# ssghost/SymbolicRegression.jl

Measured on AMD Instinct MI355X. Metric: node·row evals/sec (Float32, 4096 trees×1M rows) at 1/2/4/8 GPUs; % VALU peak, higher is better.
Workload: dtype f32

## Files before the change

symbolicregression.jl_amd/csrc/jit.cpp:

```cpp
#include "jit.h"

#include <elf.h>

#include <algorithm>
#include <chrono>
#include <cmath>
#include <cstdarg>
#include <cstdio>
#include <cstdlib>
#include <cstring>
#include <atomic>
#include <functional>
#include <mutex>
#include <thread>
#include <unordered_map>

#include "jit_asm.h"

#define HIP_CHECK(expr)                                                                  \
  do {                                                                                   \
    hipError_t _e = (expr);                                                              \
    if (_e != hipSuccess)                                                                \
      throw Error(SRHIP_ERR_DEVICE, std::string(#expr) + ": " + hipGetErrorString(_e));  \
  } while (0)
// ... 240 lines not shown
}

struct Gen {
  Asm& as;
  const Tmpl& T;
  uint64_t base_va;
  bool fast_opt;
  std::vector<IrOp> ops;
  Opnd root;
  bool fast = false;
  bool g_can = false, g_min = false, g_exp = false, g_trig = false, has_trig = false, has_call = false;
  enum { L_NONE = -1, L_A = 100, L_B = 101 };
  std::vector<int> loc;
  int pool_owner[NPOOL];
  int a_owner = -1, b_owner = -1;
  int xblk[256];
  int xlast[256];
  bool xinl[256];
  bool xdirect = false;
  std::vector<int> feats;
  int load_idx[256];
  int nloads = 0, waited = 0;
  std::vector<int> next_call;
  int L_tile = -1, L_done = -1, L_redo = -1, L_bail = -1;
  std::string why;
  bool out = false;
  int out_rreg = -1;
  int gbase = 1 << 30;
  bool gwaited = true;
  int gidx[256];
  int gnum = 0, gdone = 0;
  bool gany = false;
  bool gprefetch = [] { const char* e = std::getenv("SRHIP_JIT_GPREFETCH"); return e && e[0] == '1'; }();
  int L_reload = -1;
  void emit_gloads() {
    as.vop2(VOP2_LSHLREV_B32, "v_lshlrev_b32_e32", VGT, K(2), VLANE4);
    as.sop2(SOP2_LSHL_B32, "s_lshl_b32", 0, S(S_TILE), K(10));
    as.sop2(SOP2_ADD_U32, "s_add_u32", 0, S(S_GCOL), S(0));
    as.sop2(SOP2_ADDC_U32, "s_addc_u32", 1, S(S_GCOL + 1), K(0));
    for (size_t j = 0; j < feats.size(); ++j) {
      const int f = feats[j];
      if (!is_g(f)) continue;
      const uint32_t g = (uint32_t)(f - gbase);
      int sb = 0;
      if (g > 0) {
        as.sop2(SOP2_MUL_I32, "s_mul_i32", 2, S(S_GSTRIDE), K(g));
        as.sop2(SOP2_MUL_HI_U32, "s_mul_hi_u32", 3, S(S_GSTRIDE), K(g));
// ... 6 lines not shown
  }
  static constexpr int S_GCOL = 36, S_GSTRIDE = 38;
  bool is_g(int v) const { return v >= gbase; }

  bool trig_full = false;
  bool manual_off = false;
  bool off_exp = false, off_trig = false, off_div = false;
  static int div_rk() {
    static const int r = [] {
      for (int k = 0; k < kNumRoutines; ++k)
        if (std::string(kRoutineName[k]) == "b_div_rk") return k;
      return -1;
    }();
    return r;
  }
  static int full_routine(int rid) {
    const std::string want = std::string(kRoutineName[rid]) + "_full";
    for (int k = 0; k < kNumRoutines; ++k)
      if (want == kRoutineName[k]) return k;
    return rid;
  }
  bool inline_ok = false;
  bool packed = true, pkmov = true;
  static constexpr int SC0 = 24, NSC = 16, SPROG = 56;
  bool memc = false;
  int loss = SRHIP_LOSS_L2;
  uint64_t lparam = 0;
  std::vector<int> cpcs;
  int cslot(const Opnd& q) {
    for (size_t k = 0; k < cpcs.size(); ++k)
      if (cpcs[k] == q.pc) return (int)k;
    cpcs.push_back(q.pc);
    return (int)cpcs.size() - 1;
  }
  int creg(const Opnd& q) const {
    for (size_t k = 0; k < cpcs.size(); ++k)
      if (cpcs[k] == q.pc) return SC0 + (int)k;
    throw Error(SRHIP_ERR_INVALID, "jit: constant without a slot");
  }
  Gen(Asm& a, const Tmpl& t, uint64_t va, bool f) : as(a), T(t), base_va(va), fast_opt(f) {
    const char* e = std::getenv("SRHIP_JIT_INLINE");
    inline_ok = e && e[0] == '1';
    const char* xd = std::getenv("SRHIP_JIT_XDIRECT");
    xdirect = !(xd && xd[0] == '0');
    const char* pk = std::getenv("SRHIP_JIT_PACKED");
    packed = !(pk && pk[0] == '0');
    const char* pm = std::getenv("SRHIP_JIT_PKMOV");
    pkmov = !(pm && pm[0] == '0');
    const char* tf = std::getenv("SRHIP_JIT_TRIG_FULL");
    trig_full = tf && tf[0] == '1';
    const char* mo = std::getenv("SRHIP_JIT_MANUAL");
    manual_off = mo && mo[0] == '0';
    if (const char* mf = std::getenv("SRHIP_JIT_MANUAL_OFF")) {
      const std::string l(mf);
      off_exp = l.find("exp") != std::string::npos;
      off_trig = l.find("trig") != std::string::npos;
      off_div = l.find("div") != std::string::npos;
    }
  }

  uint64_t cur_va() const { return base_va + as.bytes(); }
  static bool trig_guard_on() {
    static const bool on = [] { const char* e = std::getenv("SRHIP_JIT_TRIG_GUARD"); return !(e && e[0] == '0'); }();
    return on;
  }
  bool trig_of_tainted(const IrOp& o) const {
    static const bool zs_only = [] { const char* e = std::getenv("SRHIP_JIT_TRIG_GUARD_ZS"); return e && e[0] == '1'; }();
    return o.un && (o.op == SRHIP_UOP_SIN || o.op == SRHIP_UOP_COS) && o.a.k == O_VAL && ops[o.a.v].taint &&
           (o.zs || !zs_only);
  }
  static bool loss_guards_on() {
    static const bool on = [] { const char* e = std::getenv("SRHIP_JIT_LOSS_GUARDS"); return !(e && e[0] == '0'); }();
    return on;
  }
  static uint32_t can_eps_bits() {
// ... 566 lines not shown
      ++nloads;
    }
    for (size_t j = 0; j < feats.size(); ++j) {
      const int f = feats[j];
      pool_owner[j] = 1000 + f;
      if (is_g(f)) continue;
      load_idx[f] = nloads++;
      as.ds_read_b128(VPOOL0 + R * (int)j, VLANE, (1 + f) * TILE * 4);
    }
    gwaited = !gany;
    gdone = 0;
    std::fill(loc.begin(), loc.end(), (int)L_NONE);
    for (int i = 0; i < (int)ops.size(); ++i) {
      if (ops[i].rid >= 0) { if (!emit_call(i)) return false; }
      else if (!emit_inline(i)) return false;
    }
    int rreg;
    if (root.k == O_VAL) rreg = reg_of_loc(loc[root.v]);
    else if (root.k == O_X) { wait_for(root); rreg = VPOOL0 + R * xblk[root.v]; }
    else {
      for (int e = 0; e < R; ++e) as.vop1(VOP1_MOV, "v_mov_b32_e32", VGT + e, memc ? S(creg(root)) : K(root.c));
      rreg = VGT;
    }
    if (packed && rreg != VGT) {
      const Src r01 = V(rreg), r23 = V(rreg + 2), z = K(0);
      as.vop3p(VOP3P_FMA_F32, "v_pk_fma_f32", VGT, r01, z, &r23, 0, 5, 0, 0);
      for (int e = 0; e < 2; ++e) {
        const Src r = V(VGT + e), c = V(VCHK);
        as.vop3(VOP3_FMA_F32, "v_fma_f32", VCHK, r, z, &c, 0, 0);
      }
    } else {
      for (int e = 0; e < R; ++e) {
        const Src r = V(rreg + e), z = K(0), c = V(VCHK);
        as.vop3(VOP3_FMA_F32, "v_fma_f32", VCHK, r, z, &c, 0, 0);
      }
    }
    wait_all();
    if (out) {
      out_rreg = rreg;
      return true;
    }
    if (fast) {
      const int L_skip = as.label();
      as.sopc(SOPC_LG_U32, "s_cmp_lg_u32", S(S_MODE), K(0));
      as.branch(SOPP_SCC1, "s_cbranch_scc1", L_skip);
      as.vopc(VOPC_U_F32, "v_cmp_u_f32_e32", V(VCHK), VCHK);
      as.branch(SOPP_VCCNZ, "s_cbranch_vccnz", L_redo);
      if (g_can) {
        as.vopc(VOPC_NGT_F32, "v_cmp_ngt_f32_e32", K(0), VGCAN);
        as.branch(SOPP_VCCNZ, "s_cbranch_vccnz", L_redo);
      }
      if (g_min) {
        as.vopc(VOPC_NLE_F32, "v_cmp_nle_f32_e32", K(0x03800000u), VGMIN);
        as.branch(SOPP_VCCNZ, "s_cbranch_vccnz", L_redo);
      }
      if (g_exp) {
        as.vopc(VOPC_NGE_F32, "v_cmp_nge_f32_e32", K(0x42ae0000u), VGEXP);
        as.branch(SOPP_VCCNZ, "s_cbranch_vccnz", L_redo);
      }
      if (g_trig) {
        static const uint32_t lim = [] {
          const char* e = std::getenv("SRHIP_JIT_TRIG_GUARD_LOG2");
          const int k = e ? std::max(1, std::min(100, std::atoi(e))) : (loss_guards_on() ? 10 : 14);
          return (uint32_t)(127 + k) << 23;
        }();
        as.vopc(VOPC_NGE_F32, "v_cmp_nge_f32_e32", K(lim), VGTRIG);
        as.branch(SOPP_VCCNZ, "s_cbranch_vccnz", L_redo);
      }
      as.bind(L_skip);
    }
    const bool margin = loss >= SRHIP_MARGIN_LOSS_BEGIN;
    if (packed) {
      Src r[R], y[R];
      for (int e = 0; e < R; ++e) { r[e] = V(rreg + e); y[e] = V(VY + e); }
      if (margin) pk_block(VOP3P_MUL_F32, "v_pk_mul_f32", VY, r, y, false);
      else pk_block(VOP3P_ADD_F32, "v_pk_add_f32", VY, r, y, true);
    } else if (margin) {
      for (int e = 0; e < R; ++e) as.vop2(VOP2_MUL_F32, "v_mul_f32_e32", VY + e, V(rreg + e), VY + e);
    } else {
      for (int e = 0; e < R; ++e) as.vop2(VOP2_SUB_F32, "v_sub_f32_e32", VY + e, V(rreg + e), VY + e);
    }
    return true;
  }

  void emit_mask(int reg) {
    const int L_nomask = as.label();
    as.sop2(SOP2_ADD_U32, "s_add_u32", S_PE, S(S_TILE), K(1));
    as.sopc(SOPC_EQ_U32, "s_cmp_eq_u32", S(S_PE), S(S_NT));
    as.branch(SOPP_SCC0, "s_cbranch_scc0", L_nomask);
    as.sopc(SOPC_EQ_U32, "s_cmp_eq_u32", S(S_PARTIAL), K((uint32_t)TILE));
    as.branch(SOPP_SCC1, "s_cbranch_scc1", L_nomask);
    for (int e = 0; e < R; ++e) {
// ... 75 lines not shown
      as.vop2(VOP2_ADD_U32, "v_add_u32_e32", VGT, S(S_WOFF), VLANE);
      as.ds_read_b128(VGT, VGT, 0);
      Src y[R], w[R];
      for (int e = 0; e < R; ++e) { y[e] = V(VY + e); w[e] = V(VGT + e); }
      if (packed) pk_block(VOP3P_MUL_F32, "v_pk_mul_f32", VY, y, y, false);
      else for (int e = 0; e < R; ++e) as.vop2(VOP2_MUL_F32, "v_mul_f32_e32", VY + e, V(VY + e), VY + e);
      as.waitcnt_lgkm(0);
      if (packed) pk_block(VOP3P_MUL_F32, "v_pk_mul_f32", VY, w, y, false);
      else for (int e = 0; e < R; ++e) as.vop2(VOP2_MUL_F32, "v_mul_f32_e32", VY + e, V(VGT + e), VY + e);
      emit_mask(VY);
      as.vop2(VOP2_ADD_F32, "v_add_f32_e32", VY, V(VY), VY + 2);
      as.vop2(VOP2_ADD_F32, "v_add_f32_e32", VY + 1, V(VY + 1), VY + 3);
      as.vop2(VOP2_ADD_F32, "v_add_f32_e32", VY, V(VY), VY + 1);
      as.vop2(VOP2_ADD_F32, "v_add_f32_e32", VLSUM, V(VLSUM), VY);
      as.branch(SOPP_BRANCH, "s_branch", L_sum);
      as.bind(L_unw);
      emit_mask(VY);
      for (int e = 0; e < R; ++e) {
        const Src r = V(VY + e), l = V(VLSUM);
        as.vop3(VOP3_FMA_F32, "v_fma_f32", VLSUM, r, r, &l, 0, 0);
      }
      as.bind(L_sum);
    }
    if (!out) {
      as.vopc(VOPC_U_F32, "v_cmp_u_f32_e32", V(VCHK), VCHK);
      as.branch(SOPP_VCCNZ, "s_cbranch_vccnz", L_done);
    }
    static const bool sticky = [] { const char* e = std::getenv("SRHIP_JIT_STICKY"); return !(e && e[0] == '0'); }();
    if (fast && !sticky) {
      const int L_keep = as.label();
      as.sopc(SOPC_EQ_U32, "s_cmp_eq_u32", S(S_FASTOK), K(0));
      as.branch(SOPP_SCC1, "s_cbranch_scc1", L_keep);
      as.sopc(SOPC_EQ_U32, "s_cmp_eq_u32", S(S_MODE), K(0));
      as.branch(SOPP_SCC1, "s_cbranch_scc1", L_keep);
      as.sop1(SOP1_MOV, "s_mov_b32", S_MODE, K(0), "s" + std::to_string(S_MODE));
      shift_base(false);
      as.bind(L_keep);
    }
    as.vop2(VOP2_ADD_U32, "v_add_u32_e32", VLANE, S(S_TILEBYTES), VLANE);
    as.sop2(SOP2_ADD_U32, "s_add_u32", S_TILE, S(S_TILE), K(1));
    as.sopc(SOPC_LT_U32, "s_cmp_lt_u32", S(S_TILE), S(S_NT));
    if (gany && gprefetch) {
      as.branch(SOPP_SCC0, "s_cbranch_scc0", L_done);
      emit_gloads();
      as.branch(SOPP_BRANCH, "s_branch", L_tile);
    } else {
      as.branch(SOPP_SCC1, "s_cbranch_scc1", L_tile);
    }
    as.bind(L_done);
    as.sop1(SOP1_SETPC, "s_setpc_b64", 0, S(S_RT), "");
    if (as.want_text) as.lines.back() = "s_setpc_b64 s[" + std::to_string(S_RT) + ":" + std::to_string(S_RT + 1) + "]";
    if (fast) {
      as.bind(L_redo);
      as.sop2(SOP2_ADD_U32, "s_add_u32", S_X0, S(S_X0), K(1));
      as.vop1(VOP1_MOV, "v_mov_b32_e32", VCHK, V(VCHKSAVE));
      as.sop1(SOP1_MOV, "s_mov_b32", S_MODE, K(1), "s" + std::to_string(S_MODE));
      shift_base(true);
      as.branch(SOPP_BRANCH, "s_branch", (gany && gprefetch) ? L_reload : L_tile);
    }
    if (has_trig) {
      as.bind(L_bail);
      as.waitcnt_lgkm(0);
      if (gany) as.waitcnt_vm(0);
      as.vop1(VOP1_MOV, "v_mov_b32_e32", VCHK, V(VCHKSAVE));
      as.sop1(SOP1_MOV, "s_mov_b32", S_STATUS, K(1), "s" + std::to_string(S_STATUS));
      as.sop1(SOP1_SETPC, "s_setpc_b64", 0, S(S_RT), "");
      if (as.want_text) as.lines.back() = "s_setpc_b64 s[" + std::to_string(S_RT) + ":" + std::to_string(S_RT + 1) + "]";
    }
  }
};

}

static bool gen_tree(const Ins<float>* prog, const Tmpl& T, bool fast_opt, bool text, std::vector<uint32_t>& out,
                     std::vector<std::string>* lines, uint64_t area_va, int32_t* off, bool* is_fast,
                     std::string* why, const DerivedMap& dm, bool memc, int loss = SRHIP_LOSS_L2,
                     uint64_t lparam = 0, bool out_mode = false) {
  std::vector<IrOp> ir;
  Opnd root;
  if (!build_ir(prog, ir, root, &dm)) { *why = "program not translatable"; return false; }
  const size_t start = (out.size() + 15) / 16 * 16;
// ... 507 lines not shown
uint32_t* bail_flags(Module* m) { return m->d_bail; }
const Columns& columns(const Module* m) { return m->cols; }
bool memc(const Module* m) { return m && m->memc; }
int nslots(const Module* m) { return m->nslots; }
int nparts(const Module* m) { return m ? (int)m->parts.size() : 0; }
void part(const Module* m, int k, int* slot0, int* nslots) {
  *slot0 = m->parts[k].slot0;
  *nslots = m->parts[k].nslots;
}

struct JitArgs {
  EvalArgs<float> e;
  const int32_t* code_off;
  uint32_t* bail;
  uint32_t* counters;
  int fast;
  int part_lds;
  int nraw, nder;
  uint32_t der[kMaxDerived];
  const float* dcols;
  int nbig, ts;
  int dyn;
  const float* gcols;
};
struct DeriveArgs {
  const float* X;
  int64_t n_pad;
  int nder;
  uint32_t der[kMaxDerived];
  float* out;
};

hipError_t launch_derive(Module* m, const float* X, int64_t n_pad, float* out, hipStream_t stream) {
  if (m->cols.nder == 0) return hipSuccess;
  DeriveArgs da;
  da.X = X;
  da.n_pad = n_pad;
  da.nder = m->cols.nder;
  std::memcpy(da.der, m->cols.der, sizeof(da.der));
  da.out = out;
  size_t sz = sizeof(da);
  void* cfg[] = {HIP_LAUNCH_PARAM_BUFFER_POINTER, &da, HIP_LAUNCH_PARAM_BUFFER_SIZE, &sz, HIP_LAUNCH_PARAM_END};
  const unsigned gx = (unsigned)std::min<int64_t>(1024, (n_pad / 4 + 255) / 256);
  return hipModuleLaunchKernel(m->parts[0].fn_derive, std::max(gx, 1u), (unsigned)m->cols.nder, 1, 256, 1, 1, 0,
                               stream, nullptr, cfg);
}

int64_t flag_words(Module* m) { return (int64_t)m->nslots + 2; }

hipError_t reset_flags(Module* m, hipStream_t stream) {
  return hipMemsetAsync(m->d_bail, 0, (size_t)(m->nslots + 2) * sizeof(uint32_t), stream);
}

bool dynamic_trees() { return false; }

static bool dynloop() {
  const char* e = std::getenv("SRHIP_JIT_DYNLOOP");
  return !(e && e[0] == '0');
}

bool partials4(Module* m, int k) {
  const ModulePart& q = m->parts[k];
  return q.fn_dl && !m->out && dynloop();
}

hipError_t launch(Module* m, int k, const EvalPlan& plan, const EvalArgs<float>& a, bool fast, const float* dcols,
                  hipStream_t stream, const float* gcols) {
  const ModulePart& q = m->parts[k];
  if (a.nlist != q.nslots) return hipErrorInvalidValue;
  if (m->out && (a.w != nullptr || a.out == nullptr || a.out_stride < a.n_pad)) return hipErrorInvalidValue;
  JitArgs ja;
  ja.e = a;
  ja.code_off = q.d_off;
  ja.bail = m->d_bail + q.slot0;
  ja.counters = m->d_bail + m->nslots;
  ja.fast = (fast && !m->out) ? 1 : 0;
  ja.nraw = m->cols.nraw;
  ja.nder = m->cols.nder;
  std::memcpy(ja.der, m->cols.der, sizeof(ja.der));
  ja.dcols = dcols;
  if (m->cols.ngcol > 0 && (!gcols || (uint64_t)a.n_pad * 4u > 0xffffffffu)) return hipErrorInvalidValue;
  ja.gcols = m->cols.ngcol > 0 ? gcols : nullptr;
  ja.nbig = plan.nbig >= 0 ? plan.nbig : a.nrg;
  ja.ts = plan.nbig >= 0 ? plan.ts : plan.ntiles;
  {
    const char* e = std::getenv("SRHIP_JIT_STICKY_TREE");
    ja.dyn = (e && e[0] == '1') ? 1 : (e && e[0] == '0') ? 0 : (a.nrg <= 48 ? 1 : 0);
  }
  if (ja.nraw > a.nfeat) return hipErrorInvalidValue;
  if (ja.nbig > a.nrg || ja.ts < 1 || ja.ts > plan.ntiles) return hipErrorInvalidValue;
  const size_t part_bytes = (size_t)a.tpb * sizeof(Part<float>);
  ja.part_lds = part_bytes <= 8192 && !part_global() ? 1 : 0;
  size_t sz = sizeof(ja);
  void* cfg[] = {HIP_LAUNCH_PARAM_BUFFER_POINTER, &ja, HIP_LAUNCH_PARAM_BUFFER_SIZE, &sz, HIP_LAUNCH_PARAM_END};
  const unsigned grid = a.rotate >= 2 ? (unsigned)((a.nrg + 7) / 8 * 8) * (unsigned)a.ntg
                                      : (unsigned)a.nrg * (unsigned)a.ntg;
  static const unsigned pad = [] { const char* e = std::getenv("SRHIP_JIT_LDS_PAD"); return e ? (unsigned)std::atoi(e) : 0u; }();
  const size_t narr = 1 + (size_t)(ja.nraw + ja.nder) + (a.w ? 1 : 0);
  const size_t lds = narr * (size_t)plan.ntiles * (size_t)plan.tile * sizeof(float) + (ja.part_lds ? part_bytes : 0) + 16;
  hipFunction_t fn = a.w ? q.fn_w : q.fn;
  if (m->out && q.fn_dl && dynloop()) fn = q.fn_dl;
  const char* name = m->out ? (m->memc ? (fn == q.fn_dl ? "sr_jit_out_md" : "sr_jit_out_m")
                                       : (fn == q.fn_dl ? "sr_jit_out_d" : "sr_jit_out"))
                            : m->memc ? (a.w ? "sr_jit_eval_mw" : "sr_jit_eval_m") : (a.w ? "sr_jit_eval_w" : "sr_jit_eval");
  if (q.fn_dl && !m->out && dynloop()) {
    fn = a.w ? q.fn_dlw : q.fn_dl;
    name = m->memc ? (a.w ? "sr_jit_eval_dlmw" : "sr_jit_eval_dlm") : (a.w ? "sr_jit_eval_dlw" : "sr_jit_eval_dl");
  }
  static const auto prefetch = [] { const char* e = std::getenv("SRHIP_JIT_PREFETCH"); return !(e && e[0] == '0'); };
  if (q.fn_dlp && !m->out && dynloop() && prefetch()) {
    fn = a.w ? q.fn_dlpw : q.fn_dlp;
// ... 9 lines not shown
```

symbolicregression.jl_amd/csrc/jit_template.hip:

```cpp
#include <hip/hip_runtime.h>

#include "interp.h"
#include "kernels.h"
#include "gen/jit_layout_r4.h"
#include "gen/jit_routines_r4.inc"

#ifndef SR_JIT_AREA_WORDS
#define SR_JIT_AREA_WORDS "65536"
#endif

using namespace srhip;
using namespace srhip::interp;

extern "C" __global__ void __launch_bounds__(64) sr_jit_routines() { asm volatile(SR_JIT_ROUTINES_TEXT); }

extern "C" __global__ void __launch_bounds__(64) sr_jit_area() {
  asm volatile("s_endpgm\n.globl sr_jit_code\n.hidden sr_jit_code\nsr_jit_code:\n.fill " SR_JIT_AREA_WORDS ", 4, 0xbf810000\n");
}

namespace {
constexpr int R = SR_JIT_R;
constexpr int TILE = 64 * R;
}

// ... 11 lines not shown
    rg = (k / a.ntg) * 8 + (b & 7);
    g = k % a.ntg;
    return rg < a.nrg;
  }
  rg = b / a.ntg;
  g = b - rg * a.ntg;
  return true;
}

struct JitArgs {
  EvalArgs<float> e;
  const int32_t* code_off;
  uint32_t* bail;
  uint32_t* counters;
  int fast;
  int part_lds;
  int nraw, nder;
  uint32_t der[48];
  const float* dcols;
  int nbig;
  int ts;
  int dyn;
  const float* gcols;
};

__device__ __forceinline__ float derive_uop(int op, float x) {
  switch (op) {
#define SR_DERIVE_CASE(U) case U: return dev::uop<U>(x);
    SR_DERIVE_CASE(SRHIP_UOP_EXP) SR_DERIVE_CASE(SRHIP_UOP_LOG) SR_DERIVE_CASE(SRHIP_UOP_LOG2)
    SR_DERIVE_CASE(SRHIP_UOP_LOG10) SR_DERIVE_CASE(SRHIP_UOP_LOG1P) SR_DERIVE_CASE(SRHIP_UOP_SQRT)
    SR_DERIVE_CASE(SRHIP_UOP_SIN) SR_DERIVE_CASE(SRHIP_UOP_COS) SR_DERIVE_CASE(SRHIP_UOP_TAN)
    SR_DERIVE_CASE(SRHIP_UOP_SINH) SR_DERIVE_CASE(SRHIP_UOP_COSH) SR_DERIVE_CASE(SRHIP_UOP_TANH)
    SR_DERIVE_CASE(SRHIP_UOP_ATAN) SR_DERIVE_CASE(SRHIP_UOP_ASINH) SR_DERIVE_CASE(SRHIP_UOP_ACOSH)
    SR_DERIVE_CASE(SRHIP_UOP_ATANH_CLIP) SR_DERIVE_CASE(SRHIP_UOP_ERF) SR_DERIVE_CASE(SRHIP_UOP_ERFC)
    SR_DERIVE_CASE(SRHIP_UOP_GAMMA) SR_DERIVE_CASE(SRHIP_UOP_RELU) SR_DERIVE_CASE(SRHIP_UOP_ROUND)
    SR_DERIVE_CASE(SRHIP_UOP_FLOOR) SR_DERIVE_CASE(SRHIP_UOP_CEIL) SR_DERIVE_CASE(SRHIP_UOP_SIGN)
    SR_DERIVE_CASE(SRHIP_UOP_INV)
#undef SR_DERIVE_CASE
    default: return __builtin_nanf("");
  }
}

__device__ __forceinline__ uint64_t sgpr64(uint64_t v) {
  return (uint64_t)(uint32_t)__builtin_amdgcn_readfirstlane((int)(uint32_t)v) |
         ((uint64_t)(uint32_t)__builtin_amdgcn_readfirstlane((int)(uint32_t)(v >> 32)) << 32);
}

// ... 140 lines not shown
    chk = __builtin_amdgcn_ballot_w64(chk != chk) != 0 ? __builtin_nanf("") : 0.0f;
    if (lane == 0) dst[i] = Part<float>{lsum, chk};
    if (!OUT && !skip && chk != chk && lane == 0)
      __hip_atomic_store(a.fail + s, 1u, __ATOMIC_RELAXED, __HIP_MEMORY_SCOPE_AGENT);
  };
  if constexpr (DYN) {
    auto claim = [&]() -> int {
      uint32_t v = 0u;
      if (lane == 0) v = __hip_atomic_fetch_add(cnt, 1u, __ATOMIC_RELAXED, __HIP_MEMORY_SCOPE_WORKGROUP);
      return __builtin_amdgcn_readfirstlane((int)v);
    };
    auto valid = [&](int i) { return i < a.tpb && slot_of(i) < a.nlist; };
    int i = claim();
    int32_t cnext = valid(i) ? code_of(slot_of(i)) : 0;
    while (valid(i)) {
      const int s = __builtin_amdgcn_readfirstlane(slot_of(i));
      const int inx = claim();
      const int32_t coff = cnext;
      if (valid(inx)) cnext = code_of(slot_of(inx));
      run_tree(i, s, false, coff);
      i = inx;
    }
  } else {
    int m = wave < a.tpb ? (a.tpb - wave + nwaves - 1) / nwaves : 0;
    while (m > 0 && slot_of(wave + (m - 1) * nwaves) >= a.nlist) --m;
    m = __builtin_amdgcn_readfirstlane(m);
    uint32_t fnext = m > 0 ? ld_flag(slot_of(wave)) : 0u;
    int32_t cnext = m > 0 ? code_of(slot_of(wave)) : 0;
    for (int k = 0; k < m; ++k) {
      const int i = __builtin_amdgcn_readfirstlane(wave + k * nwaves);
      const int s = __builtin_amdgcn_readfirstlane(slot_of(i));
      const bool more = k + 1 < m;
      const bool skip = __builtin_amdgcn_readfirstlane((int)fnext) != 0;
      const int32_t coff = cnext;
      if (more) {
        fnext = ld_flag(slot_of(wave + (k + 1) * nwaves));
        cnext = code_of(slot_of(wave + (k + 1) * nwaves));
      }
      run_tree(i, s, skip, coff);
    }
  }
  if (lane == 0 && __builtin_amdgcn_readfirstlane((int)redos) != 0)
    __hip_atomic_fetch_add(ja.counters + 1, (uint32_t)__builtin_amdgcn_readfirstlane((int)redos),
                           __ATOMIC_RELAXED, __HIP_MEMORY_SCOPE_AGENT);
  if (ja.part_lds) {
    __syncthreads();
    for (int i = threadIdx.x; i < a.tpb; i += nthreads) gdst[i] = sPart[i];
  }
}

struct DeriveArgs {
  const float* X;
  int64_t n_pad;
  int nder;
  uint32_t der[48];
  float* out;
};
extern "C" __global__ void __launch_bounds__(256) sr_jit_derive(DeriveArgs da) {
  const int k = blockIdx.y;
  const uint32_t d = da.der[k];
  const int op = (int)(d >> 16);
  const float* x = da.X + (size_t)(d & 0xffffu) * da.n_pad;
  float* o = da.out + (size_t)k * da.n_pad;
  for (int64_t i = (int64_t)blockIdx.x * blockDim.x + threadIdx.x; i < da.n_pad / 4; i += (int64_t)gridDim.x * blockDim.x) {
    const float4 v = reinterpret_cast<const float4*>(x)[i];
    reinterpret_cast<float4*>(o)[i] = make_float4(derive_uop(op, v.x), derive_uop(op, v.y), derive_uop(op, v.z),
                                                  derive_uop(op, v.w));
  }
}

extern "C" __global__ void __launch_bounds__(1024) sr_jit_eval(JitArgs ja) { jit_eval_body<false, false>(ja); }
extern "C" __global__ void __launch_bounds__(1024) sr_jit_eval_w(JitArgs ja) { jit_eval_body<true, false>(ja); }
extern "C" __global__ void __launch_bounds__(1024) sr_jit_eval_m(JitArgs ja) { jit_eval_body<false, true>(ja); }
extern "C" __global__ void __launch_bounds__(1024) sr_jit_eval_mw(JitArgs ja) { jit_eval_body<true, true>(ja); }
extern "C" __global__ void __launch_bounds__(1024) sr_jit_out(JitArgs ja) { jit_eval_body<false, false, true>(ja); }
extern "C" __global__ void __launch_bounds__(1024) sr_jit_out_m(JitArgs ja) { jit_eval_body<false, true, true>(ja); }
extern "C" __global__ void __launch_bounds__(1024) sr_jit_out_d(JitArgs ja) { jit_eval_body<false, false, true, true>(ja); }
extern "C" __global__ void __launch_bounds__(1024) sr_jit_out_md(JitArgs ja) { jit_eval_body<false, true, true, true>(ja); }

#define SR_JIT_LOOP_TEXT(NAME, PROG)                                                              \
  ".globl " #NAME "\n.hidden " #NAME "\n.p2align 6\n" #NAME ":\n"               \
  "v_mov_b32_e32 v89, 1\n"                                                            \
  ".L" #NAME "_next:\n"                                                                     \
  "s_mov_b64 s[58:59], exec\n"                                                        \
  "s_mov_b64 exec, 1\n"                                                               \
  "ds_add_rtn_u32 v90, v31, v89\n"                                                    \
  "s_waitcnt lgkmcnt(0)\n"                                                            \
  "s_mov_b64 exec, s[58:59]\n"                                                        \
  "v_readlane_b32 s60, v90, 0\n"                                                      \
  "s_cmp_ge_u32 s60, s40\n"                                                           \
  "s_cbranch_scc1 .L" #NAME "_done\n"                                                       \
  "s_mul_i32 s61, s60, s41\n"                                                         \
  "s_bitcmp1_b32 s60, 0\n"                                                            \
  "s_cselect_b32 s62, s43, s42\n"                                                     \
  "s_add_u32 s61, s61, s62\n"                                                         \
  "s_cmp_ge_u32 s61, s44\n"                                                           \
  "s_cbranch_scc1 .L" #NAME "_done\n"                                                       \
  "s_lshl_b32 s62, s61, 2\n"                                                          \
  "v_mov_b32_e32 v90, s62\n"                                                          \
  "global_load_dword v91, v90, s[46:47] sc1\n"                                        \
  "s_load_dword s63, s[48:49], s62\n"                                                 \
  "s_waitcnt vmcnt(0) lgkmcnt(0)\n"                                                   \
  "v_readfirstlane_b32 s62, v91\n"                                                    \
  "s_cmp_lg_u32 s62, 0\n"                                                             \
  "s_cbranch_scc1 .L" #NAME "_skip\n"                                                       \
  "s_add_u32 s96, s88, s63\n"                                                         \
  "s_addc_u32 s97, s89, 0\n"                                                          \
  PROG                                                                                \
  "v_mov_b32_e32 v41, v30\n"                                                          \
  "v_mov_b32_e32 v42, 0\n"                                                            \
  "v_mov_b32_e32 v40, 0\n"                                                            \
  "s_mov_b32 s64, 0\n"                                                                \
  "s_swappc_b64 s[76:77], s[96:97]\n"                                                 \
  "v_mov_b32_e32 v89, 1\n"                                                            \
  "s_cmp_eq_u32 s69, 0\n"                                                             \
  "s_cbranch_scc1 .L" #NAME "_sum\n"                                                        \
  "v_mov_b32_e32 v40, 0x7fc00000\n"                                                   \
  "s_mov_b64 s[58:59], exec\n"                                                        \
  "s_mov_b64 exec, 1\n"                                                               \
  "s_lshl_b32 s62, s61, 2\n"                                                          \
// ... 49 lines not shown
  ".L" #NAME "_skip:\n"                                                                     \
  "s_mov_b64 s[58:59], exec\n"                                                        \
  "s_mov_b64 exec, 1\n"                                                               \
  "v_mov_b32_e32 v0, 0\n"                                                             \
  "s_lshl_b32 s62, s60, 2\n"                                                          \
  "s_cmp_eq_u32 s52, 0\n"                                                             \
  "s_cbranch_scc1 .L" #NAME "_g2\n"                                                         \
  "v_mov_b32_e32 v2, s53\n"                                                           \
  "v_add_u32_e32 v2, s62, v2\n"                                                       \
  "ds_write_b32 v2, v0\n"                                                         \
  "s_branch .L" #NAME "_st2\n"                                                              \
  ".L" #NAME "_g2:\n"                                                                       \
  "v_mov_b32_e32 v2, s62\n"                                                           \
  "global_store_dword v2, v0, s[50:51]\n"                                       \
  ".L" #NAME "_st2:\n"                                                                      \
  "s_mov_b64 exec, s[58:59]\n"                                                        \
  "s_branch .L" #NAME "_next\n"                                                             \
  ".L" #NAME "_done:\n"                                                                     \
  "s_waitcnt vmcnt(0) lgkmcnt(0)\n"                                                   \
  "s_setpc_b64 s[94:95]\n"
#define SR_JIT_LOOP_PF_TEXT(NAME)                                                      \
  ".globl " #NAME "\n.hidden " #NAME "\n.p2align 6\n" #NAME ":\n"               \
  "v_mov_b32_e32 v89, 1\n"                                                       \
  "s_mov_b64 s[96:97], exec\n"                                                   \
  "s_mov_b64 exec, 1\n"                                                          \
  "ds_add_rtn_u32 v90, v31, v89\n"                                               \
  "s_waitcnt lgkmcnt(0)\n"                                                       \
  "s_mov_b64 exec, s[96:97]\n"                                                   \
  "v_readlane_b32 s58, v90, 0\n"                                                 \
  "s_cmp_ge_u32 s58, s40\n"                                                      \
  "s_cbranch_scc1 .L" #NAME "_inv0\n"                                        \
  "s_mul_i32 s59, s58, s41\n"                                                    \
  "s_bitcmp1_b32 s58, 0\n"                                                       \
  "s_cselect_b32 s62, s43, s42\n"                                                \
  "s_add_u32 s59, s59, s62\n"                                                    \
  "s_cmp_ge_u32 s59, s44\n"                                                      \
  "s_cbranch_scc1 .L" #NAME "_inv0\n"                                        \
  "s_lshl_b32 s62, s59, 2\n"                                                     \
  "v_mov_b32_e32 v90, s62\n"                                                     \
  "global_load_dword v92, v90, s[46:47] sc1\n"                                   \
  "s_load_dword s23, s[48:49], s62\n"                                            \
  "s_branch .L" #NAME "_ok0\n"                                        \
  ".L" #NAME "_inv0:\n"                                        \
  "s_mov_b32 s58, -1\n"                                                          \
  ".L" #NAME "_ok0:\n"                                        \
  ".L" #NAME "_next:\n"                                        \
  "s_cmp_ge_u32 s58, s40\n"                                                      \
  "s_cbranch_scc1 .L" #NAME "_done\n"                                        \
  "s_waitcnt vmcnt(0) lgkmcnt(0)\n"                                              \
  "v_readfirstlane_b32 s62, v92\n"                                               \
  "s_mov_b32 s60, s58\n"                                                         \
  "s_mov_b32 s61, s59\n"                                                         \
  "s_mov_b32 s63, s23\n"                                                         \
  "s_mov_b32 s91, s62\n"                                                         \
  "s_mov_b64 s[96:97], exec\n"                                                   \
  "s_mov_b64 exec, 1\n"                                                          \
  "ds_add_rtn_u32 v90, v31, v89\n"                                               \
  "s_waitcnt lgkmcnt(0)\n"                                                       \
  "s_mov_b64 exec, s[96:97]\n"                                                   \
  "v_readlane_b32 s58, v90, 0\n"                                                 \
  "s_cmp_ge_u32 s58, s40\n"                                                      \
  "s_cbranch_scc1 .L" #NAME "_inv1\n"                                        \
  "s_mul_i32 s59, s58, s41\n"                                                    \
  "s_bitcmp1_b32 s58, 0\n"                                                       \
  "s_cselect_b32 s62, s43, s42\n"                                                \
  "s_add_u32 s59, s59, s62\n"                                                    \
  "s_cmp_ge_u32 s59, s44\n"                                                      \
  "s_cbranch_scc1 .L" #NAME "_inv1\n"                                        \
  "s_lshl_b32 s62, s59, 2\n"                                                     \
  "v_mov_b32_e32 v90, s62\n"                                                     \
  "global_load_dword v92, v90, s[46:47] sc1\n"                                   \
  "s_load_dword s23, s[48:49], s62\n"                                            \
  "s_branch .L" #NAME "_ok1\n"                                        \
  ".L" #NAME "_inv1:\n"                                        \
  "s_mov_b32 s58, -1\n"                                                          \
  ".L" #NAME "_ok1:\n"                                        \
  "s_bitcmp1_b32 s91, 0\n"                                                       \
  "s_cbranch_scc1 .L" #NAME "_skip\n"                                        \
  "s_and_b32 s79, s45, 1\n"                                                          \
  "s_bitcmp1_b32 s91, 1\n"                                                           \
  "s_cselect_b32 s79, 0, s79\n"                                                      \
  "s_mov_b32 s91, s84\n"                                                             \
  "s_add_u32 s96, s88, s63\n"                                                         \
  "s_addc_u32 s97, s89, 0\n"                                                          \
  "v_mov_b32_e32 v41, v30\n"                                                          \
  "v_mov_b32_e32 v42, 0\n"                                                            \
  "v_mov_b32_e32 v40, 0\n"                                                            \
  "s_mov_b32 s64, 0\n"                                                                \
  "s_swappc_b64 s[76:77], s[96:97]\n"                                                 \
  "v_mov_b32_e32 v89, 1\n"                                                            \
  "s_cmp_eq_u32 s84, s91\n"                                                          \
// ... 73 lines not shown
  "v_mov_b32_e32 v2, s53\n"                                                           \
  "v_add_u32_e32 v2, s62, v2\n"                                                       \
  "ds_write_b32 v2, v0\n"                                                         \
  "s_branch .L" #NAME "_st2\n"                                                              \
  ".L" #NAME "_g2:\n"                                                                       \
  "v_mov_b32_e32 v2, s62\n"                                                           \
  "global_store_dword v2, v0, s[50:51]\n"                                       \
  ".L" #NAME "_st2:\n"                                                                      \
  "s_mov_b64 exec, s[96:97]\n"                                                        \
  "s_branch .L" #NAME "_next\n"                                                             \
  ".L" #NAME "_done:\n"                                                                     \
  "s_waitcnt vmcnt(0) lgkmcnt(0)\n"                                                   \
  "s_setpc_b64 s[94:95]\n"


#define SR_JIT_LOOP_PROG                                                              \
  "s_lshl_b32 s62, s61, 2\n"                                                          \
  "s_load_dword s91, s[100:101], s62\n"                                               \
  "s_waitcnt lgkmcnt(0)\n"                                                            \
  "s_lshl_b32 s91, s91, 3\n"                                                          \
  "s_add_u32 s56, s98, s91\n"                                                         \
  "s_addc_u32 s57, s99, 0\n"
extern "C" __global__ void __launch_bounds__(64) sr_jit_loop_holder() {
  asm volatile("s_endpgm\n" SR_JIT_LOOP_TEXT(sr_jit_loop, "") SR_JIT_LOOP_TEXT(sr_jit_loop_m, SR_JIT_LOOP_PROG)
                   SR_JIT_LOOP_PF_TEXT(sr_jit_loop_p));
}

template <bool W, bool MEMC, bool PF = false>
__device__ __forceinline__ void jit_eval_dl_body(const JitArgs& ja) {
  const EvalArgs<float>& a = ja.e;
  extern __shared__ __attribute__((aligned(16))) unsigned char smem[];
  float* sX = reinterpret_cast<float*>(smem);
  const int ncol = ja.nraw + ja.nder;
  const int narr = 1 + ncol + (W ? 1 : 0);
  const int rows = a.ntiles * TILE;
  int rg, g;
  if (!block_of(a, rg, g)) return;
  const bool tail = rg >= ja.nbig;
  const int ntl = tail ? ja.ts : a.ntiles;
  const int64_t row0 = tail ? (int64_t)ja.nbig * rows + (int64_t)(rg - ja.nbig) * ja.ts * TILE : (int64_t)rg * rows;
  const int nthreads = __builtin_amdgcn_readfirstlane((int)blockDim.x);
  float* gdst = reinterpret_cast<float*>(a.partial) + (size_t)rg * ((size_t)a.ntg * a.tpb) + (size_t)g * a.tpb;
  Part<float>* sPart = reinterpret_cast<Part<float>*>(sX + (size_t)narr * rows);
  uint32_t* cnt = reinterpret_cast<uint32_t*>(reinterpret_cast<unsigned char*>(sPart) +
                                              (ja.part_lds ? (size_t)a.tpb * sizeof(Part<float>) : 0));
  {
    constexpr int V = TILE / 4;
// ... 36 lines not shown
      "s_add_u32 s88, s88, sr_jit_code@rel32@lo+4\n"
      "s_addc_u32 s89, s89, sr_jit_code@rel32@hi+12"
      : "={s[88:89]}"(area)
      :
      : "scc");
  const uint32_t lds_lane = (uint32_t)reinterpret_cast<uintptr_t>((const __attribute__((address_space(3))) float*)sX) +
                            (uint32_t)lane * 16u;
  const uint32_t cnt_addr = (uint32_t)reinterpret_cast<uintptr_t>((const __attribute__((address_space(3))) uint32_t*)cnt);
  const uint32_t spart = (uint32_t)reinterpret_cast<uintptr_t>((const __attribute__((address_space(3))) Part<float>*)sPart);
  const uint32_t tilebytes = (uint32_t)(narr * TILE * 4);
  const uint32_t woff = W ? (uint32_t)((1 + ncol) * TILE * 4) : 0u;
  const uint32_t lane4 = (uint32_t)lane * R;
  const uint32_t partial = (uint32_t)last_valid;
  const uint32_t nt_u = (uint32_t)nt_valid;
  const uint32_t fastok = (uint32_t)ja.fast;
  const uint32_t tpb = (uint32_t)a.tpb, ntg = (uint32_t)a.ntg, gg = (uint32_t)g, g1 = (uint32_t)(a.ntg - 1 - g);
  const uint32_t nlist = (uint32_t)a.nlist, plds = (uint32_t)ja.part_lds;
  const uint64_t failp = reinterpret_cast<uint64_t>(a.fail), codep = reinterpret_cast<uint64_t>(ja.code_off);
  const uint64_t dstp = reinterpret_cast<uint64_t>(gdst), bailp = reinterpret_cast<uint64_t>(ja.bail);
  const uint64_t cntp = reinterpret_cast<uint64_t>(ja.counters);
  const uint64_t gcb = sgpr64(ja.gcols ? reinterpret_cast<uint64_t>(ja.gcols + row0) : 0ull);
  const uint32_t gstride = (uint32_t)__builtin_amdgcn_readfirstlane((int)(uint32_t)(a.n_pad * 4));
  uint32_t redos = 0;
  if constexpr (MEMC) {
    const uint64_t progp = reinterpret_cast<uint64_t>(a.prog), lop = reinterpret_cast<uint64_t>(a.list_off);
    asm volatile(
        "s_getpc_b64 s[96:97]\n"
        "s_add_u32 s96, s96, sr_jit_loop_m@rel32@lo+4\n"
        "s_addc_u32 s97, s97, sr_jit_loop_m@rel32@hi+12\n"
        "s_swappc_b64 s[94:95], s[96:97]"
        : "+{s84}"(redos)
        : "{v30}"(lds_lane), "{v31}"(cnt_addr), "{v43}"(lane4), "{s65}"(nt_u), "{s66}"(partial), "{s67}"(tilebytes),
          "{s68}"(woff), "{s79}"(fastok), "{s40}"(tpb), "{s41}"(ntg), "{s42}"(gg), "{s43}"(g1), "{s44}"(nlist),
          "{s[46:47]}"(failp), "{s[48:49]}"(codep), "{s[50:51]}"(dstp), "{s52}"(plds), "{s53}"(spart),
          "{s[54:55]}"(bailp), "{s[92:93]}"(cntp), "{s[88:89]}"(area), "{s[98:99]}"(progp), "{s[100:101]}"(lop)
        : SR_JIT_CLOBBERS_MEMC, "s56", "s57", "s58", "s59", "s60", "s61", "s62", "s63", "s64", "s69", "s91", "s94",
          "s95", "s96", "s97", "v40", "v41", "v42", "v89", "v90", "v91", "memory");
  } else if constexpr (PF) {
    const uint32_t fastflags = fastok | (ja.dyn ? 2u : 0u);
    asm volatile(
        "s_getpc_b64 s[96:97]\n"
        "s_add_u32 s96, s96, sr_jit_loop_p@rel32@lo+4\n"
        "s_addc_u32 s97, s97, sr_jit_loop_p@rel32@hi+12\n"
        "s_swappc_b64 s[94:95], s[96:97]"
        : "+{s84}"(redos)
        : "{v30}"(lds_lane), "{v31}"(cnt_addr), "{v43}"(lane4), "{s65}"(nt_u), "{s66}"(partial), "{s67}"(tilebytes),
          "{s68}"(woff), "{s45}"(fastflags), "{s40}"(tpb), "{s41}"(ntg), "{s42}"(gg), "{s43}"(g1), "{s44}"(nlist),
          "{s[46:47]}"(failp), "{s[48:49]}"(codep), "{s[50:51]}"(dstp), "{s52}"(plds), "{s53}"(spart),
          "{s[54:55]}"(bailp), "{s[92:93]}"(cntp), "{s[88:89]}"(area), "{s[36:37]}"(gcb), "{s38}"(gstride)
        : SR_JIT_CLOBBERS, "s23", "s58", "s59", "s60", "s61", "s62", "s63", "s64", "s69", "s79", "s91", "s94", "s95",
          "s96", "s97", "v40", "v41", "v42", "v89", "v90", "v91", "v92", "memory");
  } else {
    asm volatile(
        "s_getpc_b64 s[96:97]\n"
        "s_add_u32 s96, s96, sr_jit_loop@rel32@lo+4\n"
        "s_addc_u32 s97, s97, sr_jit_loop@rel32@hi+12\n"
        "s_swappc_b64 s[94:95], s[96:97]"
        : "+{s84}"(redos)
        : "{v30}"(lds_lane), "{v31}"(cnt_addr), "{v43}"(lane4), "{s65}"(nt_u), "{s66}"(partial), "{s67}"(tilebytes),
          "{s68}"(woff), "{s79}"(fastok), "{s40}"(tpb), "{s41}"(ntg), "{s42}"(gg), "{s43}"(g1), "{s44}"(nlist),
          "{s[46:47]}"(failp), "{s[48:49]}"(codep), "{s[50:51]}"(dstp), "{s52}"(plds), "{s53}"(spart),
          "{s[54:55]}"(bailp), "{s[92:93]}"(cntp), "{s[88:89]}"(area), "{s[36:37]}"(gcb), "{s38}"(gstride)
        : SR_JIT_CLOBBERS, "s58", "s59", "s60", "s61", "s62", "s63", "s64", "s69", "s91", "s94", "s95", "s96", "s97",
          "v40", "v41", "v42", "v89", "v90", "v91", "memory");
  }
  if (lane == 0 && __builtin_amdgcn_readfirstlane((int)redos) != 0)
    __hip_atomic_fetch_add(ja.counters + 1, (uint32_t)__builtin_amdgcn_readfirstlane((int)redos),
                           __ATOMIC_RELAXED, __HIP_MEMORY_SCOPE_AGENT);
  if (ja.part_lds) {
    __syncthreads();
    const float* sPart4 = reinterpret_cast<const float*>(sPart);
    for (int i = threadIdx.x; i < a.tpb; i += nthreads) gdst[i] = sPart4[i];
  }
}
extern "C" __global__ void __launch_bounds__(1024) sr_jit_eval_dl(JitArgs ja) { jit_eval_dl_body<false, false>(ja); }
extern "C" __global__ void __launch_bounds__(1024) sr_jit_eval_dlw(JitArgs ja) { jit_eval_dl_body<true, false>(ja); }
extern "C" __global__ void __launch_bounds__(1024) sr_jit_eval_dlp(JitArgs ja) { jit_eval_dl_body<false, false, true>(ja); }
extern "C" __global__ void __launch_bounds__(1024) sr_jit_eval_dlpw(JitArgs ja) { jit_eval_dl_body<true, false, true>(ja); }
extern "C" __global__ void __launch_bounds__(1024) sr_jit_eval_dlm(JitArgs ja) { jit_eval_dl_body<false, true>(ja); }
extern "C" __global__ void __launch_bounds__(1024) sr_jit_eval_dlmw(JitArgs ja) { jit_eval_dl_body<true, true>(ja); }

struct JitGradArgs {
  EvalArgs<float> e;
  const int32_t* code_off;
  const float* consts;
// ... 263 lines not shown
```

Measured before the change: 25140 billion.

## Rotate per-row-group tree start order and trim root NaN check sequence

Each resident row group now starts claiming trees at a rotated offset (rg*rot_step mod tpb). The goal is to spread concurrent workgroups across different trees and cut contention and imbalance on shared tree code and flags. Invalid slots now skip to the next claim instead of ending the loop. Separately, the root checksum is built with two packed FMAs, and one unordered compare feeds a direct fail path that writes NaN and returns, which drops the per-element FMA chain and the later L2 NaN check. Risks include a changed tree visiting order, register pressure from the new SGPR inputs (s45/s98), and possible correctness issues in the new early-fail path.

```diff
diff --git a/symbolicregression.jl_amd/csrc/jit.cpp b/symbolicregression.jl_amd/csrc/jit.cpp
--- a/symbolicregression.jl_amd/csrc/jit.cpp
+++ b/symbolicregression.jl_amd/csrc/jit.cpp
@@ -286,7 +286,7 @@
   int load_idx[256];
   int nloads = 0, waited = 0;
   std::vector<int> next_call;
-  int L_tile = -1, L_done = -1, L_redo = -1, L_bail = -1;
+  int L_tile = -1, L_done = -1, L_redo = -1, L_bail = -1, L_fail = -1;
   std::string why;
   bool out = false;
   int out_rreg = -1;
@@ -339,6 +339,8 @@
   }
   bool inline_ok = false;
   bool packed = true, pkmov = true;
+  bool trim_root = true;
+  bool root2 = false;
   static constexpr int SC0 = 24, NSC = 16, SPROG = 56;
   bool memc = false;
   int loss = SRHIP_LOSS_L2;
@@ -368,6 +370,8 @@
     trig_full = tf && tf[0] == '1';
     const char* mo = std::getenv("SRHIP_JIT_MANUAL");
     manual_off = mo && mo[0] == '0';
+    const char* tr = std::getenv("SRHIP_JIT_TRIM_ROOT");
+    trim_root = !(tr && tr[0] == '0');
     if (const char* mf = std::getenv("SRHIP_JIT_MANUAL_OFF")) {
       const std::string l(mf);
       off_exp = l.find("exp") != std::string::npos;
@@ -980,7 +984,12 @@
       for (int e = 0; e < R; ++e) as.vop1(VOP1_MOV, "v_mov_b32_e32", VGT + e, memc ? S(creg(root)) : K(root.c));
       rreg = VGT;
     }
-    if (packed && rreg != VGT) {
+    root2 = trim_root && packed && rreg != VGT && !out;
+    if (root2) {
+      const Src r01 = V(rreg), r23 = V(rreg + 2), z = K(0), c = V(VCHK), t = V(VGT);
+      as.vop3p(VOP3P_FMA_F32, "v_pk_fma_f32", VGT, r01, z, &c, 0, 1, 0, 0);
+      as.vop3p(VOP3P_FMA_F32, "v_pk_fma_f32", VGT, r23, z, &t, 0, 5, 0, 0);
+    } else if (packed && rreg != VGT) {
       const Src r01 = V(rreg), r23 = V(rreg + 2), z = K(0);
       as.vop3p(VOP3P_FMA_F32, "v_pk_fma_f32", VGT, r01, z, &r23, 0, 5, 0, 0);
       for (int e = 0; e < 2; ++e) {
@@ -998,11 +1007,12 @@
       out_rreg = rreg;
       return true;
     }
+    if (root2) as.vopc(VOPC_U_F32, "v_cmp_u_f32_e32", V(VGT), VGT + 1);
     if (fast) {
       const int L_skip = as.label();
       as.sopc(SOPC_LG_U32, "s_cmp_lg_u32", S(S_MODE), K(0));
       as.branch(SOPP_SCC1, "s_cbranch_scc1", L_skip);
-      as.vopc(VOPC_U_F32, "v_cmp_u_f32_e32", V(VCHK), VCHK);
+      if (!root2) as.vopc(VOPC_U_F32, "v_cmp_u_f32_e32", V(VCHK), VCHK);
       as.branch(SOPP_VCCNZ, "s_cbranch_vccnz", L_redo);
       if (g_can) {
         as.vopc(VOPC_NGT_F32, "v_cmp_ngt_f32_e32", K(0), VGCAN);
@@ -1026,6 +1036,10 @@
         as.branch(SOPP_VCCNZ, "s_cbranch_vccnz", L_redo);
       }
       as.bind(L_skip);
+    }
+    if (root2) {
+      L_fail = as.label();
+      as.branch(SOPP_VCCNZ, "s_cbranch_vccnz", L_fail);
     }
     const bool margin = loss >= SRHIP_MARGIN_LOSS_BEGIN;
     if (packed) {
@@ -1147,7 +1161,7 @@
       }
       as.bind(L_sum);
     }
-    if (!out) {
+    if (!out && !(root2 && loss == SRHIP_LOSS_L2)) {
       as.vopc(VOPC_U_F32, "v_cmp_u_f32_e32", V(VCHK), VCHK);
       as.branch(SOPP_VCCNZ, "s_cbranch_vccnz", L_done);
     }
@@ -1182,6 +1196,12 @@
       as.sop1(SOP1_MOV, "s_mov_b32", S_MODE, K(1), "s" + std::to_string(S_MODE));
       shift_base(true);
       as.branch(SOPP_BRANCH, "s_branch", (gany && gprefetch) ? L_reload : L_tile);
+    }
+    if (root2) {
+      as.bind(L_fail);
+      as.vop1(VOP1_MOV, "v_mov_b32_e32", VCHK, K(0x7fc00000u));
+      as.sop1(SOP1_SETPC, "s_setpc_b64", 0, S(S_RT), "");
+      if (as.want_text) as.lines.back() = "s_setpc_b64 s[" + std::to_string(S_RT) + ":" + std::to_string(S_RT + 1) + "]";
     }
     if (has_trig) {
       as.bind(L_bail);
@@ -1735,6 +1755,7 @@
   int nbig, ts;
   int dyn;
   const float* gcols;
+  int rot_step, rot_nrg;
 };
 struct DeriveArgs {
   const float* X;
@@ -1771,6 +1792,8 @@
   const char* e = std::getenv("SRHIP_JIT_DYNLOOP");
   return !(e && e[0] == '0');
 }
+
+constexpr int kRotateDefault = 1;
 
 bool partials4(Module* m, int k) {
   const ModulePart& q = m->parts[k];
@@ -1800,6 +1823,25 @@
     const char* e = std::getenv("SRHIP_JIT_STICKY_TREE");
     ja.dyn = (e && e[0] == '1') ? 1 : (e && e[0] == '0') ? 0 : (a.nrg <= 48 ? 1 : 0);
   }
+  ja.rot_step = 0;
+  ja.rot_nrg = 0;
+  if (!m->out && a.tpb > 1 && a.ntg > 0) {
+    const char* e = std::getenv("SRHIP_JIT_ROTATE");
+    const int mode = e ? std::atoi(e) : kRotateDefault;
+    if (mode == 1 || mode == 2) {
+      static const int ncu = [] {
+        int dev = 0, n = 0;
+        if (hipGetDevice(&dev) != hipSuccess ||
+            hipDeviceGetAttribute(&n, hipDeviceAttributeMultiprocessorCount, dev) != hipSuccess || n < 1)
+          n = 256;
+        return n;
+      }();
+      const int per_cu = std::max(1, 20 / std::max(1, plan.threads / 64));
+      const int resident = std::max(1, std::min(a.nrg, ncu * per_cu / a.ntg));
+      ja.rot_step = std::max(1, a.tpb / resident);
+      ja.rot_nrg = mode == 2 ? a.nrg : resident;
+    }
+  }
   if (ja.nraw > a.nfeat) return hipErrorInvalidValue;
   if (ja.nbig > a.nrg || ja.ts < 1 || ja.ts > plan.ntiles) return hipErrorInvalidValue;
   const size_t part_bytes = (size_t)a.tpb * sizeof(Part<float>);
diff --git a/symbolicregression.jl_amd/csrc/jit_template.hip b/symbolicregression.jl_amd/csrc/jit_template.hip
--- a/symbolicregression.jl_amd/csrc/jit_template.hip
+++ b/symbolicregression.jl_amd/csrc/jit_template.hip
@@ -57,7 +57,13 @@
   int ts;
   int dyn;
   const float* gcols;
+  int rot_step, rot_nrg;
 };
+
+__device__ __forceinline__ uint32_t rot_of(const JitArgs& ja, int rg) {
+  if (ja.rot_step <= 0 || rg >= ja.rot_nrg) return 0u;
+  return (uint32_t)__builtin_amdgcn_readfirstlane((int)(((int64_t)rg * ja.rot_step) % ja.e.tpb));
+}
 
 __device__ __forceinline__ float derive_uop(int op, float x) {
   switch (op) {
@@ -244,22 +250,31 @@
       i = inx;
     }
   } else {
-    int m = wave < a.tpb ? (a.tpb - wave + nwaves - 1) / nwaves : 0;
-    while (m > 0 && slot_of(wave + (m - 1) * nwaves) >= a.nlist) --m;
-    m = __builtin_amdgcn_readfirstlane(m);
-    uint32_t fnext = m > 0 ? ld_flag(slot_of(wave)) : 0u;
-    int32_t cnext = m > 0 ? code_of(slot_of(wave)) : 0;
-    for (int k = 0; k < m; ++k) {
-      const int i = __builtin_amdgcn_readfirstlane(wave + k * nwaves);
+    const int m = __builtin_amdgcn_readfirstlane(wave < a.tpb ? (a.tpb - wave + nwaves - 1) / nwaves : 0);
+    const int rot = OUT ? 0 : (int)rot_of(ja, rg);
+    auto pos_of = [&](int k) {
+      const int i = wave + k * nwaves + rot;
+      return i >= a.tpb ? i - a.tpb : i;
+    };
+    auto next_valid = [&](int k) {
+      while (k < m && slot_of(pos_of(k)) >= a.nlist) ++k;
+      return __builtin_amdgcn_readfirstlane(k);
+    };
+    int k = next_valid(0);
+    uint32_t fnext = k < m ? ld_flag(slot_of(pos_of(k))) : 0u;
+    int32_t cnext = k < m ? code_of(slot_of(pos_of(k))) : 0;
+    while (k < m) {
+      const int i = __builtin_amdgcn_readfirstlane(pos_of(k));
       const int s = __builtin_amdgcn_readfirstlane(slot_of(i));
-      const bool more = k + 1 < m;
+      const int k2 = next_valid(k + 1);
       const bool skip = __builtin_amdgcn_readfirstlane((int)fnext) != 0;
       const int32_t coff = cnext;
-      if (more) {
-        fnext = ld_flag(slot_of(wave + (k + 1) * nwaves));
-        cnext = code_of(slot_of(wave + (k + 1) * nwaves));
+      if (k2 < m) {
+        fnext = ld_flag(slot_of(pos_of(k2)));
+        cnext = code_of(slot_of(pos_of(k2)));
       }
       run_tree(i, s, skip, coff);
+      k = k2;
     }
   }
   if (lane == 0 && __builtin_amdgcn_readfirstlane((int)redos) != 0)
@@ -300,7 +315,7 @@
 extern "C" __global__ void __launch_bounds__(1024) sr_jit_out_d(JitArgs ja) { jit_eval_body<false, false, true, true>(ja); }
 extern "C" __global__ void __launch_bounds__(1024) sr_jit_out_md(JitArgs ja) { jit_eval_body<false, true, true, true>(ja); }
 
-#define SR_JIT_LOOP_TEXT(NAME, PROG)                                                              \
+#define SR_JIT_LOOP_TEXT(NAME, PROG, ROT)                                                         \
   ".globl " #NAME "\n.hidden " #NAME "\n.p2align 6\n" #NAME ":\n"               \
   "v_mov_b32_e32 v89, 1\n"                                                            \
   ".L" #NAME "_next:\n"                                                                     \
@@ -312,12 +327,16 @@
   "v_readlane_b32 s60, v90, 0\n"                                                      \
   "s_cmp_ge_u32 s60, s40\n"                                                           \
   "s_cbranch_scc1 .L" #NAME "_done\n"                                                       \
+  "s_add_u32 s60, s60, " ROT "\n"                                                     \
+  "s_sub_u32 s62, s60, s40\n"                                                         \
+  "s_cmp_ge_u32 s60, s40\n"                                                           \
+  "s_cselect_b32 s60, s62, s60\n"                                                     \
   "s_mul_i32 s61, s60, s41\n"                                                         \
   "s_bitcmp1_b32 s60, 0\n"                                                            \
   "s_cselect_b32 s62, s43, s42\n"                                                     \
   "s_add_u32 s61, s61, s62\n"                                                         \
   "s_cmp_ge_u32 s61, s44\n"                                                           \
-  "s_cbranch_scc1 .L" #NAME "_done\n"                                                       \
+  "s_cbranch_scc1 .L" #NAME "_next\n"                                                       \
   "s_lshl_b32 s62, s61, 2\n"                                                          \
   "v_mov_b32_e32 v90, s62\n"                                                          \
   "global_load_dword v91, v90, s[46:47] sc1\n"                                        \
@@ -413,6 +432,7 @@
 #define SR_JIT_LOOP_PF_TEXT(NAME)                                                      \
   ".globl " #NAME "\n.hidden " #NAME "\n.p2align 6\n" #NAME ":\n"               \
   "v_mov_b32_e32 v89, 1\n"                                                       \
+  ".L" #NAME "_claim0:\n"                                                   \
   "s_mov_b64 s[96:97], exec\n"                                                   \
   "s_mov_b64 exec, 1\n"                                                          \
   "ds_add_rtn_u32 v90, v31, v89\n"                                               \
@@ -421,12 +441,16 @@
   "v_readlane_b32 s58, v90, 0\n"                                                 \
   "s_cmp_ge_u32 s58, s40\n"                                                      \
   "s_cbranch_scc1 .L" #NAME "_inv0\n"                                        \
+  "s_add_u32 s58, s58, s98\n"                                                    \
+  "s_sub_u32 s62, s58, s40\n"                                                    \
+  "s_cmp_ge_u32 s58, s40\n"                                                      \
+  "s_cselect_b32 s58, s62, s58\n"                                                \
   "s_mul_i32 s59, s58, s41\n"                                                    \
   "s_bitcmp1_b32 s58, 0\n"                                                       \
   "s_cselect_b32 s62, s43, s42\n"                                                \
   "s_add_u32 s59, s59, s62\n"                                                    \
   "s_cmp_ge_u32 s59, s44\n"                                                      \
-  "s_cbranch_scc1 .L" #NAME "_inv0\n"                                        \
+  "s_cbranch_scc1 .L" #NAME "_claim0\n"                                      \
   "s_lshl_b32 s62, s59, 2\n"                                                     \
   "v_mov_b32_e32 v90, s62\n"                                                     \
   "global_load_dword v92, v90, s[46:47] sc1\n"                                   \
@@ -444,6 +468,7 @@
   "s_mov_b32 s61, s59\n"                                                         \
   "s_mov_b32 s63, s23\n"                                                         \
   "s_mov_b32 s91, s62\n"                                                         \
+  ".L" #NAME "_claim1:\n"                                                   \
   "s_mov_b64 s[96:97], exec\n"                                                   \
   "s_mov_b64 exec, 1\n"                                                          \
   "ds_add_rtn_u32 v90, v31, v89\n"                                               \
@@ -452,12 +477,16 @@
   "v_readlane_b32 s58, v90, 0\n"                                                 \
   "s_cmp_ge_u32 s58, s40\n"                                                      \
   "s_cbranch_scc1 .L" #NAME "_inv1\n"                                        \
+  "s_add_u32 s58, s58, s98\n"                                                    \
+  "s_sub_u32 s62, s58, s40\n"                                                    \
+  "s_cmp_ge_u32 s58, s40\n"                                                      \
+  "s_cselect_b32 s58, s62, s58\n"                                                \
   "s_mul_i32 s59, s58, s41\n"                                                    \
   "s_bitcmp1_b32 s58, 0\n"                                                       \
   "s_cselect_b32 s62, s43, s42\n"                                                \
   "s_add_u32 s59, s59, s62\n"                                                    \
   "s_cmp_ge_u32 s59, s44\n"                                                      \
-  "s_cbranch_scc1 .L" #NAME "_inv1\n"                                        \
+  "s_cbranch_scc1 .L" #NAME "_claim1\n"                                      \
   "s_lshl_b32 s62, s59, 2\n"                                                     \
   "v_mov_b32_e32 v90, s62\n"                                                     \
   "global_load_dword v92, v90, s[46:47] sc1\n"                                   \
@@ -577,7 +606,7 @@
   "s_add_u32 s56, s98, s91\n"                                                         \
   "s_addc_u32 s57, s99, 0\n"
 extern "C" __global__ void __launch_bounds__(64) sr_jit_loop_holder() {
-  asm volatile("s_endpgm\n" SR_JIT_LOOP_TEXT(sr_jit_loop, "") SR_JIT_LOOP_TEXT(sr_jit_loop_m, SR_JIT_LOOP_PROG)
+  asm volatile("s_endpgm\n" SR_JIT_LOOP_TEXT(sr_jit_loop, "", "s45") SR_JIT_LOOP_TEXT(sr_jit_loop_m, SR_JIT_LOOP_PROG, "s45")
                    SR_JIT_LOOP_PF_TEXT(sr_jit_loop_p));
 }
 
@@ -660,6 +689,7 @@
   const uint64_t gcb = sgpr64(ja.gcols ? reinterpret_cast<uint64_t>(ja.gcols + row0) : 0ull);
   const uint32_t gstride = (uint32_t)__builtin_amdgcn_readfirstlane((int)(uint32_t)(a.n_pad * 4));
   uint32_t redos = 0;
+  const uint32_t rot = rot_of(ja, rg);
   if constexpr (MEMC) {
     const uint64_t progp = reinterpret_cast<uint64_t>(a.prog), lop = reinterpret_cast<uint64_t>(a.list_off);
     asm volatile(
@@ -671,7 +701,8 @@
         : "{v30}"(lds_lane), "{v31}"(cnt_addr), "{v43}"(lane4), "{s65}"(nt_u), "{s66}"(partial), "{s67}"(tilebytes),
           "{s68}"(woff), "{s79}"(fastok), "{s40}"(tpb), "{s41}"(ntg), "{s42}"(gg), "{s43}"(g1), "{s44}"(nlist),
           "{s[46:47]}"(failp), "{s[48:49]}"(codep), "{s[50:51]}"(dstp), "{s52}"(plds), "{s53}"(spart),
-          "{s[54:55]}"(bailp), "{s[92:93]}"(cntp), "{s[88:89]}"(area), "{s[98:99]}"(progp), "{s[100:101]}"(lop)
+          "{s[54:55]}"(bailp), "{s[92:93]}"(cntp), "{s[88:89]}"(area), "{s[98:99]}"(progp), "{s[100:101]}"(lop),
+          "{s45}"(rot)
         : SR_JIT_CLOBBERS_MEMC, "s56", "s57", "s58", "s59", "s60", "s61", "s62", "s63", "s64", "s69", "s91", "s94",
           "s95", "s96", "s97", "v40", "v41", "v42", "v89", "v90", "v91", "memory");
   } else if constexpr (PF) {
@@ -685,7 +716,8 @@
         : "{v30}"(lds_lane), "{v31}"(cnt_addr), "{v43}"(lane4), "{s65}"(nt_u), "{s66}"(partial), "{s67}"(tilebytes),
           "{s68}"(woff), "{s45}"(fastflags), "{s40}"(tpb), "{s41}"(ntg), "{s42}"(gg), "{s43}"(g1), "{s44}"(nlist),
           "{s[46:47]}"(failp), "{s[48:49]}"(codep), "{s[50:51]}"(dstp), "{s52}"(plds), "{s53}"(spart),
-          "{s[54:55]}"(bailp), "{s[92:93]}"(cntp), "{s[88:89]}"(area), "{s[36:37]}"(gcb), "{s38}"(gstride)
+          "{s[54:55]}"(bailp), "{s[92:93]}"(cntp), "{s[88:89]}"(area), "{s[36:37]}"(gcb), "{s38}"(gstride),
+          "{s98}"(rot)
         : SR_JIT_CLOBBERS, "s23", "s58", "s59", "s60", "s61", "s62", "s63", "s64", "s69", "s79", "s91", "s94", "s95",
           "s96", "s97", "v40", "v41", "v42", "v89", "v90", "v91", "v92", "memory");
   } else {
@@ -698,7 +730,8 @@
         : "{v30}"(lds_lane), "{v31}"(cnt_addr), "{v43}"(lane4), "{s65}"(nt_u), "{s66}"(partial), "{s67}"(tilebytes),
           "{s68}"(woff), "{s79}"(fastok), "{s40}"(tpb), "{s41}"(ntg), "{s42}"(gg), "{s43}"(g1), "{s44}"(nlist),
           "{s[46:47]}"(failp), "{s[48:49]}"(codep), "{s[50:51]}"(dstp), "{s52}"(plds), "{s53}"(spart),
-          "{s[54:55]}"(bailp), "{s[92:93]}"(cntp), "{s[88:89]}"(area), "{s[36:37]}"(gcb), "{s38}"(gstride)
+          "{s[54:55]}"(bailp), "{s[92:93]}"(cntp), "{s[88:89]}"(area), "{s[36:37]}"(gcb), "{s38}"(gstride),
+          "{s45}"(rot)
         : SR_JIT_CLOBBERS, "s58", "s59", "s60", "s61", "s62", "s63", "s64", "s69", "s91", "s94", "s95", "s96", "s97",
           "v40", "v41", "v42", "v89", "v90", "v91", "memory");
   }
```

Result: faster. 25900 billion (median of 6 runs) (+3.1%).
